# lhoyer/improving_segmentation_with_selfsupervised_depth

Measured on AMD Instinct MI355X. Metric: train images/sec, ResNet-101 joint seg+depth @512x1024, higher is better.
Workload: dtype f32

## Files before the change

### improving_segmentation_with_selfsupervised_depth_amd/_lib.py

```python
import ctypes
import os
from ctypes import c_int, c_long, c_float, c_void_p, c_size_t, c_uint64, c_int64, POINTER

_HERE = os.path.dirname(os.path.abspath(__file__))
LIB_PATH = os.environ.get("SEGSDE_LIB") or os.path.join(_HERE, "libsegsde_hip.so")
ABI_VERSION = 21

_LIB = None
HOST_POINTERS_OK = False


class PackJob(ctypes.Structure):
    _fields_ = [("w", c_void_p), ("fwd", c_void_p), ("dgrad", c_void_p)] + [(n, c_int) for n in (
        "O", "I", "KH", "KW", "block0", "reserved")]


class WinoJob(ctypes.Structure):
    _fields_ = [("w", c_void_p), ("u_fwd", c_void_p), ("u_dgrad", c_void_p)] + [(n, c_int) for n in ("O", "I", "block0", "reserved")]


class BnFoldJob(ctypes.Structure):
    _fields_ = [(n, c_void_p) for n in ("w", "cb", "gamma", "beta", "mean", "var", "w_out", "b_out")] + [("eps", c_float)] + [
        (n, c_int) for n in ("O", "I", "KH", "KW", "block0", "reserved")]

# ... 5 lines not shown


P = c_void_p
_SIGS = {
    "segsde_abi_version": (c_int, []),
    "segsde_conv_compute_taken": (c_int, [POINTER(ConvDesc), c_int]),
    "segsde_split_bf16_planes": (c_int, [P, c_long, P, P, P, P]),
    "segsde_conv2d_forward": (c_int, [POINTER(ConvDesc), P, P, P, P, P, P, P]),
    "segsde_conv2d_stats_rows": (c_long, [POINTER(ConvDesc)]),
    "segsde_conv2d_forward_stats": (c_int, [POINTER(ConvDesc), P, P, P, P, P, P, P, P]),
    "segsde_conv2d_dgrad_actgrad": (c_int, [POINTER(ConvDesc), P, P, P, P, P, P, P, P, c_int, c_int, P]),
    "segsde_bn_stats_from_partials_workspace": (c_size_t, [c_int]),
    "segsde_bn_stats_from_partials": (c_int, [P, c_long, c_long, c_int, P, P, P, P, c_float, c_float, P, P, c_size_t, P]),
    "segsde_conv2d_forward_residual": (c_int, [POINTER(ConvDesc), P, P, P, P, P, c_int, P, P]),
    "segsde_conv2d_wgrad_workspace": (c_size_t, [POINTER(ConvDesc)]),
    "segsde_conv2d_wgrad": (c_int, [POINTER(ConvDesc), P, P, P, c_int, P, P, c_size_t, P]),
    "segsde_conv2d_winograd_workspace": (c_size_t, [POINTER(ConvDesc)]),
    "segsde_conv2d_winograd_stats_rows": (ctypes.c_long, [POINTER(ConvDesc)]),
    "segsde_winograd_pack": (c_int, [P, c_int, c_int, P, P, P]),
    "segsde_winograd_pack_multi": (c_int, [P, c_int, c_int, P]),
    "segsde_conv2d_winograd": (c_int, [POINTER(ConvDesc), P, P, P, P, P, P, P, P, c_size_t, P]),
    "segsde_conv2d_wgrad_winograd_workspace": (c_size_t, [POINTER(ConvDesc)]),
    "segsde_conv2d_wgrad_winograd": (c_int, [POINTER(ConvDesc), P, P, P, c_int, P, P, P, c_size_t, P]),
    "segsde_winograd_fused_ok": (c_int, [c_int, c_int, c_int, c_int, c_int]),
    "segsde_winograd_fused_stats_rows": (ctypes.c_long, [c_int, c_int, c_int]),
    "segsde_winograd_fused_pack": (c_int, [P, c_int, c_int, c_int, P, P]),
    "segsde_conv2d_winograd_fused": (c_int, [P, c_int, c_int, c_int, c_int, c_int, c_int, P, c_int, P, c_int, P, c_int, c_int, P, P]),
    "segsde_conv2d_winograd_fused2": (c_int, [P, c_int, c_int, c_int, P, c_int, c_int, c_int, c_int, c_int, c_int, P, c_int, P, c_int, P,
                                              c_int, P, P]),
    "segsde_conv2d_winograd_fused_dgrad": (c_int, [P, c_int, c_int, c_int, c_int, c_int, P, c_int, c_int, P, c_int, c_int, P, c_int, c_int, P]),
    "segsde_reflect_adjoint_borders": (c_int, [P, P, P, P, P, c_int, c_int, P]),
    "segsde_reflect_adjoint_borders_ok": (c_int, [P, c_int]),
    "segsde_reflect_adjoint_borders2": (c_int, [P, c_int, P, c_int, P, c_int, P, c_int, c_int, c_int, c_int, c_int, c_int, c_int, P]),
    "segsde_conv2d_wgrad_winograd_fused_workspace": (c_size_t, [P]),
    "segsde_conv2d_wgrad_winograd_fused": (c_int, [P, P, P, P, c_int, P, P, c_size_t, P]),
    "segsde_upfold_pack": (c_int, [P, c_int, c_int, c_int, P, P, P]),
    "segsde_conv2d_forward_upfold": (c_int, [POINTER(ConvDesc), P, P, P, P, P, P, P]),
    "segsde_conv2d_dgrad_upfold": (c_int, [POINTER(ConvDesc), P, c_int, P, P, P, P, P, c_int, P, c_int, c_int, P]),
    "segsde_conv2d_wgrad_upfold_workspace": (c_size_t, [POINTER(ConvDesc)]),
    "segsde_conv2d_wgrad_upfold": (c_int, [POINTER(ConvDesc), P, P, P, c_int, P, P, c_size_t, P]),
    "segsde_stem_pack": (c_int, [P, c_int, c_int, c_int, P, P]),
    "segsde_stem7x7_stats_rows": (c_long, [c_int, c_int, c_int, c_int, c_int]),
    "segsde_stem7x7_forward": (c_int, [P, c_int, c_int, c_int, c_int, P, c_int, P, P, P]),
    "segsde_stem7x7_forward_bias_act": (c_int, [P, c_int, c_int, c_int, c_int, P, c_int, P, c_int, P, P]),
    "segsde_stem7x7_wgrad_workspace": (c_size_t, [c_int, c_int, c_int, c_int, c_int]),
    "segsde_stem7x7_wgrad": (c_int, [P, c_int, c_int, c_int, c_int, P, c_int, c_int, c_int, P, P, c_size_t, P]),
    "segsde_nchw_to_nhwc_bordered": (c_int, [P, c_int, c_int, c_int, c_int, c_float, c_float, P, c_int, c_int, c_int, c_int, c_int, P]),
    "segsde_pack_weight": (c_int, [P, P, c_int, c_int, c_int, c_int, c_int, P]),
    "segsde_pack_weight_both": (c_int, [P, P, P, c_int, c_int, c_int, c_int, P]),
    "segsde_pack_weight_both_multi": (c_int, [P, c_int, c_int, P]),
    "segsde_reflect_dgrad_fix": (c_int, [P, c_int, P, P, c_int, P, c_int, c_int, c_int, c_int, c_int, c_int, c_int, P]),
    "segsde_bn_stats_workspace": (c_size_t, [c_long, c_int]),
    "segsde_bn_stats": (c_int, [P, c_int, c_long, c_int, P, P, P, P, c_float, c_float, P, P, c_size_t, P]),
    "segsde_bn_eval_stats": (c_int, [P, P, c_int, c_float, P, P, P]),
    "segsde_bn_fold": (c_int, [P, c_int, c_int, P]),
    "segsde_bn_apply": (c_int, [P, c_int, c_long, c_int, P, P, P, P, P, c_int, P, c_int, c_int, c_float, c_uint64, P]),
    "segsde_bn_backward_workspace": (c_size_t, [c_long, c_int]),
    "segsde_bn_backward": (c_int, [P, c_int, P, c_int, P, c_int, c_long, c_int, P, P, P, P, c_int, c_float, c_uint64, c_int,
                                   P, P, P, c_int, P, c_int, P, c_size_t, P]),
    "segsde_bn_mask_words": (c_size_t, [c_long, c_int]),
    "segsde_bn_apply_mask": (c_int, [P, c_int, c_long, c_int, P, P, P, P, P, c_int, P, c_int, c_int, c_float, c_uint64, P, P]),
    "segsde_bn_backward_mask": (c_int, [P, c_int, P, P, c_int, c_long, c_int, P, P, P, c_int, c_float, c_int, P, P, P, c_int, P, c_int,
                                        P, c_size_t, P]),
    "segsde_colsum_workspace": (c_size_t, [c_long, c_int]),
    "segsde_act_backward": (c_int, [P, c_int, P, c_int, c_long, c_int, c_int, P, c_int, P, P, c_size_t, P]),
    "segsde_colsum": (c_int, [P, c_int, c_long, c_int, P, P, c_size_t, P]),
# ... 120 lines not shown
```

### improving_segmentation_with_selfsupervised_depth_amd/csrc/winograd_fused.hip

```cpp
#include <stdlib.h>
#include <type_traits>
#include "segsde_common.h"
#include "winograd.h"
#ifndef WINO_UP_SKIP
#define WINO_UP_SKIP 1
#endif

namespace {
#define ST(s) static_cast<hipStream_t>(s)
constexpr int FT_H = 4, FT_W = 8;
constexpr int FP_H = 2 * FT_H + 2, FP_W = 2 * FT_W + 2;
constexpr int FROW = 20, FODD = FP_W / 2;
constexpr int FPS = 256;
__device__ __forceinline__ constexpr int fplane(int c) { return c * FPS + 2 * (c >> 2); }
constexpr int FCH = 64;
constexpr int FZP = 36;
constexpr int F_FLOATS = 8 * 64 * FZP > FCH * FPS ? 8 * 64 * FZP : FCH * FPS;
#ifdef WINO_DBG_OCC1
constexpr size_t F_LDS = 96 * 1024;
#else
constexpr size_t F_LDS = (size_t)F_FLOATS * sizeof(float) + 2 * 4 * 64 * sizeof(double);
#endif

struct WinoSrc { const float* x0; const float* x1; int ld0, ld1, C0, up0; };
// ... 359 lines not shown
    }
  }
}

struct BorderP {
  const float* dy; const float* wp ; float* dx; const float* agy;
  int lddy, lddx, agld, agkind, B, H, W, Cin, Cout, mode, nseg, ldw;
};

__global__ __launch_bounds__(256) void reflect_borders_kernel(BorderP p) {
  SEGSDE_SMEM;
  float* sh = reinterpret_cast<float*>(segsde_smem);
  const int tid = threadIdx.x, lane = tid & 63, wave = tid >> 6, m = lane & 31, kk = lane >> 5;
  const int L = p.mode == 0 ? p.W : p.H;
  int r = blockIdx.x;
  const int seg = r % p.nseg; r /= p.nseg;
  const int far = r & 1, b = r >> 1;
  const int p0 = seg * 32, pitch = p.Cout + 1, cq4 = p.Cout >> 2;
  const int fixed = p.mode == 0 ? (far ? p.H - 1 : 0) : (far ? p.W - 1 : 0);
  for (int idx = tid; idx < 34 * cq4; idx += 256) {
    const int px = idx / cq4, q = idx - px * cq4, pos = p0 - 1 + px;
    float4 v = make_float4(0.f, 0.f, 0.f, 0.f);
    if (pos >= 0 && pos < L) {
      const long pix = p.mode == 0 ? ((long)(b * p.H + fixed) * p.W + pos) : ((long)(b * p.H + pos) * p.W + fixed);
      v = *reinterpret_cast<const float4*>(p.dy + pix * p.lddy + 4 * q);
    }
    float* d = sh + px * pitch + 4 * q;
    d[0] = v.x; d[1] = v.y; d[2] = v.z; d[3] = v.w;
  }
  __syncthreads();
  const int ktap = far ? 2 : 0;
  const bool top = p.mode == 1 && p0 <= 1 && 1 < p0 + 32, bot = p.mode == 1 && p0 <= p.H - 2 && p.H - 2 < p0 + 32;
  const int steps = p.Cout >> 1;
  for (int nb = wave; nb < (p.Cin >> 5); nb += 4) {
    const int cin = nb * 32 + m;
    f32x16 acc;
#pragma unroll
    for (int q = 0; q < 16; ++q) acc[q] = 0.f;
    for (int t = 0; t < 5; ++t) {
      if (t == 3 && !top) continue;
      if (t == 4 && !bot) continue;
      int kh, kw, src; bool mine = true;
      if (t < 3) {
        kh = p.mode == 0 ? ktap : t; kw = p.mode == 0 ? t : ktap; src = m + 2 - t;
      } else {
        kh = t == 3 ? 0 : 2; kw = ktap;
        const int at = t == 3 ? 1 : p.H - 2;
        mine = p0 + m == at;
        src = (t == 3 ? 0 : p.H - 1) - (p0 - 1);
      }
      const float* ap = sh + src * pitch + kk;
      const float* bp = p.wp + ((long)kk * 9 + kh * 3 + kw) * p.ldw + cin;
      const long bstep = 18L * p.ldw;
      float bv[2][8];
#pragma unroll
      for (int u = 0; u < 8; ++u) bv[0][u] = u < steps ? bp[u * bstep] : 0.f;
      for (int s0 = 0; s0 < steps; s0 += 16) {
#pragma unroll
        for (int half = 0; half < 2; ++half) {
          const int sb = s0 + 8 * half;
          if (sb < steps) {
#pragma unroll
            for (int u = 0; u < 8; ++u) bv[half ^ 1][u] = sb + 8 + u < steps ? bp[(long)(sb + 8 + u) * bstep] : 0.f;
#pragma unroll
            for (int u = 0; u < 8; ++u) {
              if (sb + u < steps) {
                const float a = mine ? ap[2 * (sb + u)] : 0.f;
// ... 78 lines not shown
                                            int Cout, const float* bias, int act, float* y, int ldy, int accumulate, double* stats,
                                            void* stream) {
  if (!x || !u_kn || !y) return SEGSDE_ERR_NULL;
  if (!segsde_winograd_fused_ok(B, H, W, C, Cout) || ldx < C || ldx % 4 != 0 || !pitch_ok(H, W, ldx) || ldy < Cout || !pitch_ok(H, W, ldy) || (accumulate && (stats || bias || act)))
    return SEGSDE_ERR_UNSUPPORTED;
  const WinoSrc src{x, nullptr, ldx, 0, C, 0};
  return launch_fused(src, B, H, W, C, reflect, u_kn, Cout, Cout, bias, act, y, ldy, accumulate, stats, WinoAg{nullptr, 0, 0}, stream);
}

extern "C" int segsde_conv2d_winograd_fused2(const float* x0, int ld0, int C0, int up0, const float* x1, int ld1, int C1, int B, int H,
                                             int W, int reflect, const float* u_kn, int Cout, const float* bias, int act, float* y,
                                             int ldy, double* stats, void* stream) {
  if (!x0 || !u_kn || !y || (C1 > 0 && !x1)) return SEGSDE_ERR_NULL;
  const int C = C0 + (C1 > 0 ? C1 : 0);
  if (!segsde_winograd_fused_ok(B, H, W, C, Cout) || C0 <= 0 || C0 % FCH || ld0 < C0 || ld0 % 4 != 0 || (C1 > 0 && (ld1 < C1 || ld1 % 4 != 0 || !pitch_ok(H, W, ld1))) ||
      !pitch_ok(H >> (up0 ? 1 : 0), W >> (up0 ? 1 : 0), ld0) || ldy < Cout || !pitch_ok(H, W, ldy))
    return SEGSDE_ERR_UNSUPPORTED;
  const WinoSrc src{x0, x1, ld0, ld1, C0, up0 ? 1 : 0};
  return launch_fused(src, B, H, W, C, reflect, u_kn, Cout, Cout, bias, act, y, ldy, 0, stats, WinoAg{nullptr, 0, 0}, stream);
}

extern "C" int segsde_conv2d_winograd_fused_dgrad(const float* dy, int lddy, int B, int H, int W, int Cout, const float* ud_kn, int ldu,
                                                  int Cin, float* dx, int lddx, int accumulate, const float* act_out, int act_ld,
                                                  int act_kind, void* stream) {
  if (!dy || !ud_kn || !dx) return SEGSDE_ERR_NULL;
  if (!segsde_winograd_fused_ok(B, H, W, Cout, Cin) || ldu < Cin || (long)16 * Cout * ldu >= (1L << 28) || lddy < Cout || lddy % 4 != 0 || !pitch_ok(H, W, lddy) || lddx < Cin || !pitch_ok(H, W, lddx) ||
      (act_out && (act_kind < SEGSDE_ACT_RELU || act_kind > SEGSDE_ACT_SIGMOID || act_ld < Cin || !pitch_ok(H, W, act_ld))))
    return SEGSDE_ERR_UNSUPPORTED;
  const WinoSrc src{dy, nullptr, lddy, 0, Cout, 0};
  return launch_fused(src, B, H, W, Cout, 0, ud_kn, ldu, Cin, nullptr, SEGSDE_ACT_NONE, dx, lddx, accumulate, nullptr,
                      WinoAg{act_out, act_ld, act_kind}, stream);
}

extern "C" int segsde_reflect_adjoint_borders2(const float* dy, int lddy, const float* wpack, int ldw, float* dx, int lddx,
                                               const float* act_out, int act_ld, int act_kind, int B, int H, int W, int Cin, int Cout,
                                               void* stream) {
  if (!dy || !wpack || !dx) return SEGSDE_ERR_NULL;
  if (B <= 0 || H < 4 || W < 4 || Cin <= 0 || Cin % 32 || ldw < Cin || Cout <= 0 || Cout % 32 || Cout > 1024 || lddy < Cout || lddy % 4 || lddx < Cin ||
      ((uintptr_t)dy & 15) || (act_out && (act_kind < SEGSDE_ACT_RELU || act_kind > SEGSDE_ACT_SIGMOID || act_ld < Cin)))
    return SEGSDE_ERR_UNSUPPORTED;
  BorderP p;
  p.dy = dy; p.wp = wpack; p.dx = dx; p.agy = act_out; p.lddy = lddy; p.lddx = lddx; p.agld = act_ld; p.agkind = act_kind;
  p.B = B; p.H = H; p.W = W; p.Cin = Cin; p.Cout = Cout; p.ldw = ldw;
  const size_t lb = (size_t)34 * (Cout + 1) * sizeof(float);
  (void)hipFuncSetAttribute(reinterpret_cast<const void*>(reflect_borders_kernel), hipFuncAttributeMaxDynamicSharedMemorySize, (int)lb);
  for (int mode = 0; mode < 2; ++mode) {
    p.mode = mode; p.nseg = ((mode == 0 ? W : H) + 31) / 32;
    hipLaunchKernelGGL(reflect_borders_kernel, dim3((unsigned)(B * 2 * p.nseg)), dim3(256), lb, ST(stream), p);
    SEGSDE_CHECK_LAUNCH();
  }
  return 0;
}
```

### improving_segmentation_with_selfsupervised_depth_amd/functional.py

```python
import collections
import weakref

import torch
from torch.autograd import Function as _TorchFunction

from . import hipops as H


class Function(_TorchFunction):

    @classmethod
    def apply(cls, *args):
        return super(_TorchFunction, cls).apply(*args)


FUSIONS = {}
BN_BITMASK = True


def _grad_dest(param):
    from . import ddp
    return ddp.grad_destination(param) if ddp._GRAD_DEST else None


# ... 144 lines not shown

    @staticmethod
    def forward(ctx, x0, x1, weight, bias, g, act, stats_out=None, grad_box=None, packs=None, x0_act=None, act_box=None,
                fold_cache=None, wino_cache=None, skip_box=None):
        ctx.grad_box = grad_box
        ctx.skip_box = skip_box
        ctx.x0_act, ctx.act_box = x0_act, act_box
        x0 = _c(x0) if x0.stride(-1) != 1 else x0
        ctx.wd = None
        ctx.wd_gen = None
        if packs is not None:
            wp, ctx.wd = packs
            ctx.wd_gen = getattr(ctx.wd, "_segsde_gen", None)
        elif ctx.needs_input_grad[0] or (x1 is not None and ctx.needs_input_grad[1]):
            wp, ctx.wd = H.pack_weight_both(weight)
        else:
            wp = H.pack_weight(weight, False)
        ctx.wp = wp if g.reflect else None
        ctx.fold = None
        ctx.wino = None
        up_f = 2 if g.up0 else 1
        kn = H.winograd_fused_ok(g, x0.shape[0], x0.shape[1] * up_f, x0.shape[2] * up_f)
        kn_d2 = (x1 is not None and g.up0 and (ctx.needs_input_grad[1])
                 and H.winograd_fused_dgrad2_ok(g, x0.shape[0], x0.shape[1] * up_f, x0.shape[2] * up_f))
        if kn or kn_d2 or (not g.up0 and H.winograd_ok(g, x0.shape[0], x0.shape[1], x0.shape[2])):
            knl = kn or kn_d2
            if (wino_cache is not None and wino_cache.get("key") is not None and wino_cache.get("key") == wino_cache.get("want")
                    and bool(wino_cache.get("kn")) == knl):
                ctx.wino = wino_cache["packs"]
            else:
                ctx.wino = H.winograd_pack(weight, kn=knl)
                if wino_cache is not None and wino_cache.get("want") is not None:
                    wino_cache["packs"], wino_cache["key"], wino_cache["kn"] = ctx.wino, wino_cache["want"], knl
        wino_f = None if (ctx.wino is None or (kn_d2 and not kn)) else ctx.wino[0]
        keep_v = wino_f is not None and not kn and ctx.needs_input_grad[2]
        H.WINO_V[0] = None
        if stats_out is not None:
            y, part = H.conv_forward(g, x0, x1, wp, bias, act, want_stats=True, wino=wino_f, keep_v=keep_v)
            stats_out.append(part)
        else:
            if H.upfold_ok(g, 4 * x0.shape[0] * x0.shape[1] * x0.shape[2]) and x0.is_contiguous() and (x1 is None or x1.is_contiguous()):
                if fold_cache is not None and fold_cache.get("key") is not None and fold_cache.get("key") == fold_cache.get("want"):
                    ctx.fold = fold_cache["fold"]
                else:
                    ctx.fold = H.upfold_pack(weight, g.C0)
                    if fold_cache is not None and fold_cache.get("want") is not None:
                        fold_cache["fold"], fold_cache["key"] = ctx.fold, fold_cache["want"]
            y = H.conv_forward(g, x0, x1, wp, bias, act, wfold=None if ctx.fold is None else ctx.fold[0], wino=wino_f, keep_v=keep_v)
        ctx.wino_v, H.WINO_V[0] = H.WINO_V[0], None
        ctx.g, ctx.act = g, act
        ctx.in_hw = (x0.shape[1] * (2 if g.up0 else 1), x0.shape[2] * (2 if g.up0 else 1))
        ctx.has_bias = bias is not None
        ctx.save_for_backward(x0, x1, weight)
        return y

    @staticmethod
    def backward(ctx, dy):
        x0, x1, weight = ctx.saved_tensors
        g = ctx.g
        dz = _c(dy)
        need_b = ctx.has_bias and ctx.needs_input_grad[3]
        dbias = None
        if need_b:
            stash = ctx.act_box.pop("dbias", None) if ctx.act_box is not None else None
            same = stash is not None and stash[0].data_ptr() == dz.data_ptr() and stash[0]._version == stash[1] == dz._version
            dbias = stash[2] if same else H.colsum(dz)
            fusion("bias_grad_from_activation_pass", bool(same))
        actgrad = (x0, ctx.x0_act) if ctx.x0_act is not None else None
        dx0 = dx1 = dw = None
        if ctx.needs_input_grad[0] or (x1 is not None and ctx.needs_input_grad[1]):
            wd = ctx.wd if ctx.wd is not None else H.pack_weight(weight, True)
            if ctx.wd_gen is not None and getattr(wd, "_segsde_gen", None) != ctx.wd_gen:
                raise RuntimeError("the weight packs of this graph were rebuilt by a later weight_pack_scope(model): a graph "
                                   "must be consumed before the next prepack of the same weights")
            dx0 = None
            box = ctx.grad_box
            if box is not None and box.get("g") is not None and x1 is None:
                dx0, dx1 = H.conv_dgrad(g, dz, wd, weight.detach(), ctx.in_hw, accumulate_into=box["g"], actgrad=actgrad,
                                        wino=None if ctx.wino is None else ctx.wino[1], wfpack=ctx.wp)
                if dx0 is not None:
                    box["fused"] = True
            if dx0 is None:
                sbox = ctx.skip_box if (x1 is not None and ctx.needs_input_grad[1]) else None
                dx0, dx1 = H.conv_dgrad(g, dz, wd, weight.detach(), ctx.in_hw, actgrad=actgrad, fold=ctx.fold,
                                        need0=ctx.needs_input_grad[0], need1=x1 is not None and ctx.needs_input_grad[1],
                                        wino=None if ctx.wino is None else ctx.wino[1],
                                        accumulate_skip_into=None if sbox is None else sbox.get("g"), wfpack=ctx.wp)
                if sbox is not None and dx1 is not None:
                    if H.SKIP_ACCUMULATED[0]:
                        sbox["fused"] = True
                    elif sbox.get("publish") and sbox.get("g") is None and dx1.is_contiguous():
                        sbox["g"] = dx1
                        sbox["fused"] = True
                if box is not None and box.get("publish") and box.get("g") is None and x1 is None and not g.up0 \
                        and dx0.is_contiguous():
                    box["g"] = dx0
                    box["fused"] = True
            if actgrad is not None and ctx.needs_input_grad[0]:
                fusion("activation_backward_in_dgrad_epilogue", bool(H.ACTGRAD_FUSED[0]))
            if not ctx.needs_input_grad[0]:
                dx0 = None
            if x1 is None or not ctx.needs_input_grad[1]:
                dx1 = None
        if ctx.needs_input_grad[2]:
            dw = H.conv_wgrad(g, x0, x1, dz, wino_v=ctx.wino_v, out=_grad_dest(weight))
            ctx.wino_v = None
        return dx0, dx1, dw, dbias, None, None, None, None, None, None, None, None, None, None


class ActGradFn(Function):

    passes = 0

    @staticmethod
    def forward(ctx, y, act, box):
        ctx.act, ctx.box = act, box
        ctx.save_for_backward(y)
        return y.view_as(y)

    @staticmethod
# ... 503 lines not shown
```

### improving_segmentation_with_selfsupervised_depth_amd/hipops.py

```python
import ctypes
import os
import threading

import numpy as np
import torch

from . import _lib
from ._lib import ConvDesc, check

ACT = {"none": 0, "relu": 1, "elu": 2, "sigmoid": 3}


class _Slot(threading.local):

    def __init__(self, default=None):
        self.default = default
        self.v = default

    def __getattr__(self, name):
        if name == "v":
            return self.__dict__.setdefault("v", self.__dict__.get("default"))
        raise AttributeError(name)

    def __getitem__(self, i):
# ... 136 lines not shown
    C1 = 0 if x1 is None else x1.shape[3]
    L = _lib.lib()
    d = ConvDesc(B=B, H=H, W=W, C0=C0, C1=C1, ld0=nhwc_ld(x0), ld1=nhwc_ld(x1) if x1 is not None else 0, up0=0, Ho=H, Wo=W,
                 Cout=Cout, ldy=Cout, ldy2=0, nsplit=0, KH=3, KW=3, stride=1, dil=g.dil, pad=g.dil,
                 pad_mode=PAD_REFLECT if reflect else PAD_ZERO, in_div=1, act=ACT[act], sum2x2=0)
    nbytes = L.segsde_conv2d_winograd_workspace(ctypes.byref(d))
    if not nbytes:
        return None
    y = torch.empty((B, H, W, Cout), dtype=torch.float32, device=x0.device)
    part = None
    if want_stats:
        part = torch.empty((int(L.segsde_conv2d_winograd_stats_rows(ctypes.byref(d))), 2, Cout), dtype=torch.float64, device=x0.device)
    ws = _ws(nbytes, x0)
    Tp = (B * (H // 2) * (W // 2) + 127) // 128 * 128
    vk = torch.empty((16, Tp, C0 + C1), dtype=torch.float32, device=x0.device) if keep_v else None
    rc = _timed(kind, flops, x0, lambda: L.segsde_conv2d_winograd(ctypes.byref(d), _p(_f32(x0)), _p(x1), _p(upack), _p(bias), _p(y),
                                                                   _p(part), _p(vk), _p(ws), nbytes, _stream(x0)), tag + " wino",
                executed=flops * 16.0 / 36.0)
    if rc == -4:
        return None
    check(rc, "conv2d_winograd")
    WINO_V[0] = vk
    WINOGRAD_TAKEN["fwd" if kind == "conv_fwd" else "dgrad"] += 1
    return y, part


WINO_FUSED = os.environ.get("SEGSDE_WINO_FUSED", "1") != "0"
WINO_FUSED_MAX_CH = int(os.environ.get("SEGSDE_WINO_FUSED_MAX_CH", "256"))
WINO_FUSED2 = os.environ.get("SEGSDE_WINO_FUSED2", "1") != "0"
WINO_UP_SKIP = os.environ.get("SEGSDE_WINO_UP_SKIP", "1") != "0"
WINO_FUSED2_MAX_CIN = int(os.environ.get("SEGSDE_WINO_FUSED2_MAX_CIN", "768"))
WINO_FUSED2_MIN_FOLD = float(os.environ.get("SEGSDE_WINO_FUSED2_MIN_FOLD", "0.6"))
WINO_FUSED_DGRAD_EXT = os.environ.get("SEGSDE_WINO_FUSED_DGRAD_EXT", "1") != "0"
WINO_FUSED_REFLECT_DGRAD_MIN_PIX = int(os.environ.get("SEGSDE_WINO_FUSED_REFLECT_DGRAD_MIN_PIX", str(1 << 17)))
WINO_FUSED_DGRAD2 = os.environ.get("SEGSDE_WINO_FUSED_DGRAD2", "1") != "0"
BORDERS2 = os.environ.get("SEGSDE_BORDERS2", "1") != "0"
WINO_FUSED_UBLK = os.environ.get("SEGSDE_WINO_FUSED_UBLK", "1") != "0"
WINO_FUSED_TAKEN = {"fwd": 0, "dgrad": 0, "fwd2": 0, "dgrad_refl": 0, "dgrad_actgrad": 0, "dgrad2": 0, "wgrad": 0}


_FUSED_SHAPE_OK = {}


def _fused_shape_ok(B, H, W, cin, cout):
    key = (B, H, W, cin, cout)
    r = _FUSED_SHAPE_OK.get(key)
    if r is None:
        r = _FUSED_SHAPE_OK[key] = bool(_lib.lib().segsde_winograd_fused_ok(B, H, W, cin, cout))
    return r


def winograd_fused_ok(g, B=None, H=None, W=None, dgrad=False):
    if g.compute == 1:
        return False
    cin, cout = (g.Cout, g.C0) if dgrad else (g.Cin, g.Cout)
    if not (WINOGRAD and WINO_FUSED and g.k == 3 and g.stride == 1 and g.dil == 1 and g.pad == 1 and g.cin_alg is None
            and cin % 64 == 0 and cout % 64 == 0):
        return False
    if g.up0 or g.C1:
        if dgrad or not (WINO_FUSED2 and g.up0 and g.C0 % 64 == 0 and cin <= WINO_FUSED2_MAX_CIN and cout <= WINO_FUSED_MAX_CH
                         and _fold_frac(g) >= WINO_FUSED2_MIN_FOLD):
            return False
    else:
        if max(cin, cout) > WINO_FUSED_MAX_CH or (dgrad and g.reflect and not WINO_FUSED_DGRAD_EXT):
            return False
    if B is None:
        return True
    return _fused_shape_ok(B, H, W, cin, cout) and 9.0 * B * H * W * cin * cout >= WINOGRAD_MIN_MACS


def winograd_fused_dgrad2_ok(g, B=None, H=None, W=None):
    if g.compute == 1:
        return False
    if not (WINOGRAD and WINO_FUSED and WINO_FUSED_DGRAD_EXT and WINO_FUSED_DGRAD2 and BORDERS2 and g.k == 3 and g.stride == 1 and g.dil == 1
            and g.pad == 1 and g.reflect and g.up0 and g.C1 and g.cin_alg is None and g.C1 % 64 == 0 and g.Cout % 64 == 0
            and g.C0 % 64 == 0
            and g.Cout <= WINO_FUSED_MAX_CH and g.Cin <= WINO_FUSED2_MAX_CIN):
        return False
    if B is None:
        return True
    return (B * H * W >= WINO_FUSED_REFLECT_DGRAD_MIN_PIX and _fused_shape_ok(B, H, W, g.Cout, g.C1)
            and 9.0 * B * H * W * g.C1 * g.Cout >= WINOGRAD_MIN_MACS)


def winograd_fused_static_ok(conv):
    if not (WINOGRAD and WINO_FUSED and conv.kernel_size == (3, 3) and conv.stride == (1, 1) and conv.padding == (1, 1)
            and conv.dilation == (1, 1) and conv.in_channels % 64 == 0 and conv.out_channels % 64 == 0):
        return False
    if max(conv.in_channels, conv.out_channels) <= WINO_FUSED_MAX_CH:
        return True
    return bool(WINO_FUSED2 and getattr(conv, "reflect", False) and conv.out_channels <= WINO_FUSED_MAX_CH
                and conv.in_channels <= WINO_FUSED2_MAX_CIN)


class _KnPack(torch.Tensor):
    """a transformed weight pack of the one-kernel route: 16 K N floats, logical shape [16][K][N], stored in the blocked order the
    kernel reads (WINO_FUSED_UBLK; the sixteen [K][N] planes with SEGSDE_WINO_FUSED_UBLK=0) -- a plain tensor with a type the
    dispatch can see; only the library's pack and convolution kernels interpret its contents"""


def _kn(t):
    return t.as_subclass(_KnPack)


def winograd_fused_pack(w_oihw, flip):
    O, I = w_oihw.shape[0], w_oihw.shape[1]
    w = _f32(w_oihw.detach()).contiguous()
    u = torch.empty((16, O, I) if flip else (16, I, O), dtype=torch.float32, device=w.device)
    check(_lib.lib().segsde_winograd_fused_pack(_p(w), O, I, 1 if flip else 0, _p(u), _stream(w)), "winograd_fused_pack")
    return _kn(u)


def winograd_fused(kind, x, u_kn, bias=None, act="none", want_stats=False, tag=None, reflect=False, accumulate_into=None, x1=None,
                   up0=False, actgrad=None, adjoint=None, cols=None):
    B, H0, W0, C0 = x.shape
    H, W = (2 * H0, 2 * W0) if up0 else (H0, W0)
    C1 = 0 if x1 is None else x1.shape[3]
    C = C0 + C1
    ldu = u_kn.shape[2]
    n_off, N = (0, ldu) if cols is None else cols
    assert u_kn.shape[1] == C and n_off + N <= ldu and (cols is None or (actgrad is not None or adjoint is not None or kind == "conv_dgrad"))
    L = _lib.lib()
    if accumulate_into is not None:
        y = accumulate_into
        if tuple(y.shape) != (B, H, W, N) or not y.is_contiguous() or bias is not None or act != "none" or want_stats:
            return None
    else:
        y = torch.empty((B, H, W, N), dtype=torch.float32, device=x.device)
    part = None
    if want_stats:
        part = torch.empty((int(L.segsde_winograd_fused_stats_rows(B, H, W)), 2, N), dtype=torch.float64, device=x.device)
    flops = 2.0 * B * H * W * C * N * 9
    tagf = (tag or "%d+%d->%d k3 s1 d1 %dx%d" % (C0, C1, N, H, W)) + " wino-fused"
    if x1 is not None or up0:
        assert accumulate_into is None and actgrad is None and adjoint is None
        rc = _timed(kind, flops, x, lambda: L.segsde_conv2d_winograd_fused2(
            _p(_f32(x)), nhwc_ld(x), C0, 1 if up0 else 0, _p(x1), nhwc_ld(x1) if x1 is not None else 0, C1, B, H, W, 1 if reflect else 0,
            _p(u_kn), N, _p(bias), ACT[act], _p(y), N, _p(part), _stream(x)), tagf,
            executed=flops * ((9.0 * C0 + 16.0 * C1) / (36.0 * (C0 + C1)) if (up0 and WINO_UP_SKIP) else 16.0 / 36.0))
        if rc == -4:
            return None
        check(rc, "conv2d_winograd_fused2")
        WINO_FUSED_TAKEN["fwd2"] += 1
        return y, part
    if actgrad is not None or adjoint is not None or cols is not None:
        assert bias is None and act == "none" and not want_stats and not reflect
        ag_y, ag_kind = (actgrad[0], ACT[actgrad[1]]) if actgrad is not None else (None, 0)
        ag_ld = nhwc_ld(ag_y) if ag_y is not None else 0
        acc = 1 if accumulate_into is not None else 0
        d = wdpack = wfpack = None
        if adjoint is not None:
            g, wdpack, wfpack = adjoint
            if wfpack is None or not BORDERS2:
                assert cols is None
                d = _borders_desc(B, H, W, C, N, nhwc_ld(x))

        def launch():
            u_off = 4 * ((n_off // 64) * 256 if WINO_FUSED_UBLK else n_off)
            rc = L.segsde_conv2d_winograd_fused_dgrad(_p(_f32(x)), nhwc_ld(x), B, H, W, C, ctypes.c_void_p(u_kn.data_ptr() + u_off), ldu,
                                                      N, _p(y), N, acc, _p(ag_y), ag_ld, ag_kind, _stream(x))
            if rc == 0 and adjoint is not None:
                if d is None:
                    rc = L.segsde_reflect_adjoint_borders2(_p(x), nhwc_ld(x), ctypes.c_void_p(wfpack.data_ptr() + 4 * n_off), wfpack.shape[3],
                                                           _p(y), N, _p(ag_y), ag_ld, ag_kind, B, H, W, N, C, _stream(x))
                else:
                    rc = L.segsde_reflect_adjoint_borders(ctypes.byref(d), _p(x), _p(wdpack), _p(y), _p(ag_y), ag_ld, ag_kind, _stream(x))
                if rc == -4:
                    raise RuntimeError("the mirrored-padding launches declined a shape the one-kernel data-gradient took: "
                                       "the zero-padded part is already in dx (hipops.conv_dgrad must gate this)")
            return rc
        rc = _timed(kind, flops, x, launch, tagf, executed=flops * 16.0 / 36.0)
        if rc == -4:
            return None
        check(rc, "conv2d_winograd_fused_dgrad")
        WINO_FUSED_TAKEN["dgrad"] += 1
        WINO_FUSED_TAKEN["dgrad_refl"] += adjoint is not None
        WINO_FUSED_TAKEN["dgrad_actgrad"] += actgrad is not None
        return y, None
    rc = _timed(kind, flops, x, lambda: L.segsde_conv2d_winograd_fused(_p(_f32(x)), nhwc_ld(x), B, H, W, C, 1 if reflect else 0, _p(u_kn), N, _p(bias),
                                                                       ACT[act], _p(y), N, 1 if accumulate_into is not None else 0, _p(part), _stream(x)),
                tagf, executed=flops * 16.0 / 36.0)
    if rc == -4:
        return None
    check(rc, "conv2d_winograd_fused")
    WINO_FUSED_TAKEN["fwd" if kind == "conv_fwd" else "dgrad"] += 1
    return y, part


def _borders_desc(B, H, W, Cout, Cin, lddy):
    return ConvDesc(B=B, H=H, W=W, C0=Cout, C1=0, ld0=lddy, ld1=0, up0=0, Ho=H, Wo=W, Cout=Cin, ldy=Cin, ldy2=0, nsplit=Cin, KH=3, KW=3,
                    stride=1, dil=1, pad=1, pad_mode=PAD_REFLECT_ADJOINT, in_div=1, act=0, sum2x2=0, accumulate=1)


def reflect_borders_ok(B, H, W, Cout, Cin, lddy, ag_ld=0):
    return bool(_lib.lib().segsde_reflect_adjoint_borders_ok(ctypes.byref(_borders_desc(B, H, W, Cout, Cin, lddy)), int(ag_ld)))


WINO_FUSED_WGRAD = os.environ.get("SEGSDE_WINO_FUSED_WGRAD", "1") != "0"
WINO_FUSED_WGRAD_MAX_CH = int(os.environ.get("SEGSDE_WINO_FUSED_WGRAD_MAX_CH", "256"))
WINO_FUSED_WGRAD_MAX_CIN2 = int(os.environ.get("SEGSDE_WINO_FUSED_WGRAD_MAX_CIN2", "768"))
WINO_FUSED_WGRAD_MIN_FOLD = float(os.environ.get("SEGSDE_WINO_FUSED_WGRAD_MIN_FOLD", "0.4"))


def winograd_fused_wgrad_ok(g, B=None, H=None, W=None):
    if g.compute == 1:
        return False
    if not (WINOGRAD and WINO_FUSED and WINO_FUSED_WGRAD and g.k == 3 and g.stride == 1 and g.dil == 1 and g.pad == 1
            and g.cin_alg is None and g.C0 % 32 == 0 and g.C1 % 32 == 0 and g.Cout % 64 == 0 and g.Cout <= WINO_FUSED_WGRAD_MAX_CH):
        return False
# ... 205 lines not shown
        r = _winograd("conv_fwd", g, x0, x1, wino, g.Cout, want_stats, flops, _tag(g, H, W), bias=bias, act=act, reflect=g.reflect,
                      keep_v=keep_v and WINOGRAD_KEEP_V)
        if r is not None:
            return r if want_stats else r[0]
    if wfold is not None and not want_stats:
        rc = _timed("conv_fwd", flops, x0, lambda: _lib.lib().segsde_conv2d_forward_upfold(
            ctypes.byref(d), _p(_f32(x0)), _p(x1), _p(wpack), _p(wfold), _p(bias), _p(y), _stream(x0)), _tag(g, H, W) + " fold",
            executed=flops * _fold_frac(g))
        if rc == 0:
            UPFOLD_TAKEN["fwd"] += 1
            _note_compute(d, 4, "fwd")
            return y
        if rc != -4:
            check(rc, "conv2d_forward_upfold")
    part = None
    if want_stats and bias is None and act == "none":
        rows = int(_lib.lib().segsde_conv2d_stats_rows(ctypes.byref(d)))
        if rows > 0:
            part = torch.empty((rows, 2, g.Cout), dtype=torch.float64, device=x0.device)
    _timed("conv_fwd", flops, x0, lambda: check(_lib.lib().segsde_conv2d_forward_stats(
        ctypes.byref(d), _p(_f32(x0)), _p(x1), _p(wpack), _p(bias), _p(y), None, _p(part), _stream(x0)), "conv2d_forward"),
        _tag(g, H, W), executed=flops_x)
    _note_compute(d, 0, "fwd")
    return (y, part) if want_stats else y


ACTGRAD_FUSED = _Slot(False)


SKIP_ACCUMULATED = _Slot(False)


def conv_dgrad(g, dy, wdpack, w_oihw, in_hw, need0=True, need1=True, accumulate_into=None, actgrad=None, fold=None, wino=None,
               accumulate_skip_into=None, wfpack=None):
    B, Ho, Wo, Cout = dy.shape
    H, W = in_hw
    assert Cout == g.Cout
    ACTGRAD_FUSED[0] = False
    SKIP_ACCUMULATED[0] = False
    dx1 = torch.empty((B, H, W, g.C1), dtype=torch.float32, device=dy.device) if g.C1 else None
    L = _lib.lib()
    flops = 2.0 * B * Ho * Wo * Cout * g.CinAlg * g.k * g.k
    ag_y, ag_ld, ag_kind = None, 0, 0
    if actgrad is not None:
        ag_y, ag_kind = actgrad[0], ACT[actgrad[1]]
        ag_ld = nhwc_ld(ag_y)

    if isinstance(wino, _KnPack):
        ext = actgrad is not None or g.reflect
        if (winograd_fused_ok(g, B, H, W, dgrad=True) and (Ho, Wo) == (H, W) and (not ext or WINO_FUSED_DGRAD_EXT)
                and (not g.reflect or B * H * W >= WINO_FUSED_REFLECT_DGRAD_MIN_PIX)
                and (not g.reflect or (wfpack is not None and BORDERS2 and H >= 4 and W >= 4 and g.C0 % 32 == 0 and Cout % 32 == 0 and Cout <= 1024)
                     or reflect_borders_ok(B, H, W, Cout, g.C0, nhwc_ld(dy), ag_ld))
                and (actgrad is None or (ag_ld % 4 == 0 and ag_y.data_ptr() % 16 == 0))):
            r = winograd_fused("conv_dgrad", dy, wino, tag=_tag(g, H, W), accumulate_into=accumulate_into, actgrad=actgrad,
                               adjoint=(g, wdpack, wfpack) if g.reflect else None)
            if r is not None:
                ACTGRAD_FUSED[0] = actgrad is not None
                return r[0], None
    elif (wino is not None and accumulate_into is None and actgrad is None and not g.reflect and g.C1 == 0
            and winograd_ok(g, B, H, W, dgrad=True) and (Ho, Wo) == (H, W)):
        r = _winograd("conv_dgrad", g, dy, None, wino, g.C0, False, flops, _tag(g, H, W))
        if r is not None:
            return r[0], None

    def desc(sum2x2, accumulate=0):
        return ConvDesc(B=B, H=Ho, W=Wo, C0=Cout, C1=0, ld0=nhwc_ld(dy), ld1=0, up0=0, Ho=H, Wo=W, Cout=g.Cin, ldy=g.C0,
                        ldy2=g.C1, nsplit=g.C0, KH=g.k, KW=g.k, stride=1, dil=g.dil, pad=(g.k - 1) * g.dil - g.pad,
                        pad_mode=PAD_REFLECT_ADJOINT if g.reflect else PAD_ZERO, in_div=g.stride, act=0, sum2x2=sum2x2,
                        accumulate=accumulate, compute=g.compute)

    def launch(d, y, y2, fuse):
        return L.segsde_conv2d_dgrad_actgrad(ctypes.byref(d), _p(_f32(dy)), None, _p(wdpack), None, _p(y), _p(y2), None,
                                             _p(ag_y) if fuse else None, ag_ld if fuse else 0, ag_kind if fuse else 0,
                                             _stream(dy))

    def finish_unfused(dx0):
        if actgrad is None or dx0 is None:
            return dx0
        dz, _ = act_backward(dx0, ag_y, actgrad[1])
        return dz

    if accumulate_into is not None:
        acc = accumulate_into
        if g.up0 or g.C1 or tuple(acc.shape) != (B, H, W, g.C0) or not acc.is_contiguous():
            return None, None
        d = desc(0, 1)
        rc = _timed("conv_dgrad", flops, dy, lambda: launch(d, acc, None, actgrad is not None), _tag(g, H, W),
                    executed=flops * _live_tap_frac(g, H, W))
        if rc == -4:
            return None, None
        check(rc, "conv2d dgrad (accumulate)")
        _note_compute(d, 1, "dgrad")
        ACTGRAD_FUSED[0] = actgrad is not None
        return acc, None
    if g.up0 and fold is not None and accumulate_into is None:
        wfold, wdfold = fold
# ... 1249 lines not shown
```

### include/segsde_hip.h

```cpp
#ifndef SEGSDE_HIP_H
#define SEGSDE_HIP_H
#include <stddef.h>
#include <stdint.h>

#ifdef __cplusplus
extern "C" {
#endif

#define SEGSDE_ABI_VERSION 21

enum { SEGSDE_ERR_NULL = -1, SEGSDE_ERR_SHAPE = -2, SEGSDE_ERR_WORKSPACE = -3, SEGSDE_ERR_UNSUPPORTED = -4 };
enum { SEGSDE_ACT_NONE = 0, SEGSDE_ACT_RELU = 1, SEGSDE_ACT_ELU = 2, SEGSDE_ACT_SIGMOID = 3 };
enum { SEGSDE_DTYPE_F32 = 0, SEGSDE_DTYPE_I64 = 1, SEGSDE_DTYPE_U8 = 2 };
enum { SEGSDE_PAD_ZERO = 0, SEGSDE_PAD_REFLECT = 1, SEGSDE_PAD_REFLECT_ADJOINT = 2 };

int segsde_abi_version(void);

typedef struct segsde_conv_desc {
  int B, H, W;
  int C0, C1;
  int ld0, ld1;
  int up0;
  int Ho, Wo, Cout;
  int ldy, ldy2, nsplit;
// ... 126 lines not shown
int segsde_nchw_to_nhwc_bordered(const float* x, int B, int C, int H, int W, float mean, float sd, float* y, int ldy, int pad_top,
                                 int pad_left, int Hp, int Wp, void* stream);
int segsde_nhwc_to_nchw(const float* x, int ldx, int B, int C, int H, int W, float* y, void* stream);

typedef struct segsde_wino_job {
  const float* w;
  float* u_fwd;
  float* u_dgrad;
  int O, I, block0, reserved;
} segsde_wino_job;
size_t segsde_conv2d_winograd_workspace(const segsde_conv_desc* d);
long segsde_conv2d_winograd_stats_rows(const segsde_conv_desc* d);
int segsde_winograd_pack(const float* w_oihw, int Cout, int Cin, float* u_fwd, float* u_dgrad, void* stream);
int segsde_winograd_pack_multi(const segsde_wino_job* jobs_device, int njobs, int total_blocks, void* stream);
int segsde_conv2d_winograd(const segsde_conv_desc* d, const float* x0, const float* x1, const float* u_pack, const float* bias,
                           float* y, double* stats, float* v_keep, void* workspace, size_t workspace_bytes, void* stream);
size_t segsde_conv2d_wgrad_winograd_workspace(const segsde_conv_desc* d);
int segsde_conv2d_wgrad_winograd(const segsde_conv_desc* d, const float* x0, const float* x1, const float* dy, int lddy,
                                 const float* v_saved, float* dw_oihw, void* workspace, size_t workspace_bytes, void* stream);
int segsde_winograd_fused_ok(int B, int H, int W, int C, int Cout);
long segsde_winograd_fused_stats_rows(int B, int H, int W);
int segsde_winograd_fused_pack(const float* w_oihw, int Cout, int Cin, int flip, float* u_kn, void* stream);
int segsde_conv2d_winograd_fused(const float* x, int ldx, int B, int H, int W, int C, int reflect, const float* u_kn, int Cout,
                                 const float* bias, int act, float* y, int ldy, int accumulate, double* stats, void* stream);
int segsde_conv2d_winograd_fused2(const float* x0, int ld0, int C0, int up0, const float* x1, int ld1, int C1, int B, int H, int W,
                                  int reflect, const float* u_kn, int Cout, const float* bias, int act, float* y, int ldy,
                                  double* stats, void* stream);
int segsde_conv2d_winograd_fused_dgrad(const float* dy, int lddy, int B, int H, int W, int Cout, const float* ud_kn, int ldu, int Cin,
                                       float* dx, int lddx, int accumulate, const float* act_out, int act_ld, int act_kind, void* stream);
int segsde_reflect_adjoint_borders(const segsde_conv_desc* d, const float* dy, const float* wdpack, float* y, const float* act_out,
                                   int act_ld, int act_kind, void* stream);
int segsde_reflect_adjoint_borders2(const float* dy, int lddy, const float* wpack, int ldw, float* dx, int lddx, const float* act_out,
                                    int act_ld, int act_kind, int B, int H, int W, int Cin, int Cout, void* stream);
int segsde_reflect_adjoint_borders_ok(const segsde_conv_desc* d, int act_ld);
size_t segsde_conv2d_wgrad_winograd_fused_workspace(const segsde_conv_desc* d);
int segsde_conv2d_wgrad_winograd_fused(const segsde_conv_desc* d, const float* x0, const float* x1, const float* dy, int lddy,
                                       float* dw_oihw, void* workspace, size_t workspace_bytes, void* stream);

int segsde_pose_matrix_forward(const float* axisangle, const float* translation, int B, int stride, int invert, float* M,
                               void* stream);
int segsde_pose_matrix_backward(const float* axisangle, const float* translation, const float* dM, int B, int stride,
                                int invert, float* daxisangle, float* dtranslation, void* stream);

int segsde_warp_forward(const float* disp, int hs, int ws, const float* inv_K, const float* K, const float* T,
                        const float* src, int B, int H, int W, float min_depth, float max_depth, float* color,
                        float* grid, float* depth, void* stream);
size_t segsde_warp_backward_workspace(int B, int H, int W);
int segsde_warp_backward(const float* gcolor, const float* disp, int hs, int ws, const float* inv_K, const float* K,
                         const float* T, const float* src, int B, int H, int W, float min_depth, float max_depth,
                         float* g_disp_up, float* gT, void* workspace, size_t workspace_bytes, void* stream);
int segsde_reprojection_error_forward(const float* pred, const float* target, int B, int H, int W, int no_ssim,
                                      float* err, long err_bstride, void* stream);
size_t segsde_reprojection_error_backward_workspace(int B, int H, int W);
int segsde_reprojection_error_backward(const float* pred, const float* target, const float* gerr, long gerr_bstride, int B,
                                       int H, int W, int no_ssim, float* gpred, void* workspace, size_t workspace_bytes,
                                       void* stream);
size_t segsde_automask_workspace(int B, int H, int W);
int segsde_automask_min_forward(const float* ident, const float* noise, const float* reproj, int n_reproj, int avg, int B,
                                int H, int W, uint8_t* sel, float* identity_selection, float* sum_out, void* workspace,
                                size_t workspace_bytes, void* stream);
int segsde_automask_min_backward(const uint8_t* sel, int n_ident, int n_reproj, int avg, int B, int H, int W, float scale,
                                 float* greproj, void* stream);
size_t segsde_smoothness_workspace(int B, int h, int w);
int segsde_smoothness_forward(const float* disp, const float* img, int B, int h, int w, float* mean_disp, float* out,
                              void* workspace, size_t workspace_bytes, void* stream);
int segsde_smoothness_backward(const float* disp, const float* img, const float* mean_disp, int B, int h, int w,
// ... 114 lines not shown
```

Measured before the change: 64.24.

## Add flat fused Winograd dgrad path for concat-input reflect convs and split border kernel

Adds a dgrad path for reflect-padded 3x3 convs with two concatenated inputs (decoder skip concat). It packs a flat fused Winograd weight, cached alongside the existing packs, and runs the fused dgrad kernel twice over column ranges, one for the main input and one for the skip input, accumulating into the skip gradient directly. The reflect-border adjoint kernel now spreads its input-channel blocks across a second grid dimension to raise parallelism. The minimum pixel threshold for fused reflect dgrad is lowered so smaller layers also take the fused path. The cost is an extra weight pack and cache entry per layer, and two kernel launches where there was one generic dgrad.

```diff
diff --git a/improving_segmentation_with_selfsupervised_depth_amd/_lib.py b/improving_segmentation_with_selfsupervised_depth_amd/_lib.py
--- a/improving_segmentation_with_selfsupervised_depth_amd/_lib.py
+++ b/improving_segmentation_with_selfsupervised_depth_amd/_lib.py
@@ -61,6 +61,8 @@
     "segsde_reflect_adjoint_borders": (c_int, [P, P, P, P, P, c_int, c_int, P]),
     "segsde_reflect_adjoint_borders_ok": (c_int, [P, c_int]),
     "segsde_reflect_adjoint_borders2": (c_int, [P, c_int, P, c_int, P, c_int, P, c_int, c_int, c_int, c_int, c_int, c_int, c_int, P]),
+    "segsde_reflect_adjoint_borders2_split": (c_int, [P, c_int, P, c_int, P, c_int, P, c_int, c_int, c_int, c_int, c_int, c_int, c_int, c_int,
+                                                      P]),
     "segsde_conv2d_wgrad_winograd_fused_workspace": (c_size_t, [P]),
     "segsde_conv2d_wgrad_winograd_fused": (c_int, [P, P, P, P, c_int, P, P, c_size_t, P]),
     "segsde_upfold_pack": (c_int, [P, c_int, c_int, c_int, P, P, P]),
diff --git a/improving_segmentation_with_selfsupervised_depth_amd/csrc/winograd_fused.hip b/improving_segmentation_with_selfsupervised_depth_amd/csrc/winograd_fused.hip
--- a/improving_segmentation_with_selfsupervised_depth_amd/csrc/winograd_fused.hip
+++ b/improving_segmentation_with_selfsupervised_depth_amd/csrc/winograd_fused.hip
@@ -415,7 +415,7 @@
   const int ktap = far ? 2 : 0;
   const bool top = p.mode == 1 && p0 <= 1 && 1 < p0 + 32, bot = p.mode == 1 && p0 <= p.H - 2 && p.H - 2 < p0 + 32;
   const int steps = p.Cout >> 1;
-  for (int nb = wave; nb < (p.Cin >> 5); nb += 4) {
+  for (int nb = 4 * blockIdx.y + wave; nb < (p.Cin >> 5); nb += 4 * gridDim.y) {
     const int cin = nb * 32 + m;
     f32x16 acc;
 #pragma unroll
@@ -560,9 +560,9 @@
                       WinoAg{act_out, act_ld, act_kind}, stream);
 }
 
-extern "C" int segsde_reflect_adjoint_borders2(const float* dy, int lddy, const float* wpack, int ldw, float* dx, int lddx,
-                                               const float* act_out, int act_ld, int act_kind, int B, int H, int W, int Cin, int Cout,
-                                               void* stream) {
+extern "C" int segsde_reflect_adjoint_borders2_split(const float* dy, int lddy, const float* wpack, int ldw, float* dx, int lddx,
+                                                     const float* act_out, int act_ld, int act_kind, int B, int H, int W, int Cin,
+                                                     int Cout, int split, void* stream) {
   if (!dy || !wpack || !dx) return SEGSDE_ERR_NULL;
   if (B <= 0 || H < 4 || W < 4 || Cin <= 0 || Cin % 32 || ldw < Cin || Cout <= 0 || Cout % 32 || Cout > 1024 || lddy < Cout || lddy % 4 || lddx < Cin ||
       ((uintptr_t)dy & 15) || (act_out && (act_kind < SEGSDE_ACT_RELU || act_kind > SEGSDE_ACT_SIGMOID || act_ld < Cin)))
@@ -572,10 +572,17 @@
   p.B = B; p.H = H; p.W = W; p.Cin = Cin; p.Cout = Cout; p.ldw = ldw;
   const size_t lb = (size_t)34 * (Cout + 1) * sizeof(float);
   (void)hipFuncSetAttribute(reinterpret_cast<const void*>(reflect_borders_kernel), hipFuncAttributeMaxDynamicSharedMemorySize, (int)lb);
+  const unsigned groups = split ? (unsigned)((Cin / 32 + 3) / 4) : 1u;
   for (int mode = 0; mode < 2; ++mode) {
     p.mode = mode; p.nseg = ((mode == 0 ? W : H) + 31) / 32;
-    hipLaunchKernelGGL(reflect_borders_kernel, dim3((unsigned)(B * 2 * p.nseg)), dim3(256), lb, ST(stream), p);
+    hipLaunchKernelGGL(reflect_borders_kernel, dim3((unsigned)(B * 2 * p.nseg), groups), dim3(256), lb, ST(stream), p);
     SEGSDE_CHECK_LAUNCH();
   }
   return 0;
 }
+
+extern "C" int segsde_reflect_adjoint_borders2(const float* dy, int lddy, const float* wpack, int ldw, float* dx, int lddx,
+                                               const float* act_out, int act_ld, int act_kind, int B, int H, int W, int Cin, int Cout,
+                                               void* stream) {
+  return segsde_reflect_adjoint_borders2_split(dy, lddy, wpack, ldw, dx, lddx, act_out, act_ld, act_kind, B, H, W, Cin, Cout, 1, stream);
+}
diff --git a/improving_segmentation_with_selfsupervised_depth_amd/functional.py b/improving_segmentation_with_selfsupervised_depth_amd/functional.py
--- a/improving_segmentation_with_selfsupervised_depth_amd/functional.py
+++ b/improving_segmentation_with_selfsupervised_depth_amd/functional.py
@@ -200,6 +200,17 @@
                 ctx.wino = H.winograd_pack(weight, kn=knl)
                 if wino_cache is not None and wino_cache.get("want") is not None:
                     wino_cache["packs"], wino_cache["key"], wino_cache["kn"] = ctx.wino, wino_cache["want"], knl
+        ctx.wino_flat = None
+        if (x1 is not None and not g.up0 and (ctx.needs_input_grad[0] or ctx.needs_input_grad[1])
+                and H.winograd_fused_dgrad2_flat_ok(g, x0.shape[0], x0.shape[1], x0.shape[2])):
+            want = wino_cache.get("want") if wino_cache is not None else None
+            hit = wino_cache.get("flat") if want is not None else None
+            if hit is not None and hit[0] == want:
+                ctx.wino_flat = hit[1]
+            else:
+                ctx.wino_flat = H.winograd_fused_pack(weight, True)
+                if want is not None:
+                    wino_cache["flat"] = (want, ctx.wino_flat)
         wino_f = None if (ctx.wino is None or (kn_d2 and not kn)) else ctx.wino[0]
         keep_v = wino_f is not None and not kn and ctx.needs_input_grad[2]
         H.WINO_V[0] = None
@@ -253,7 +264,8 @@
                 dx0, dx1 = H.conv_dgrad(g, dz, wd, weight.detach(), ctx.in_hw, actgrad=actgrad, fold=ctx.fold,
                                         need0=ctx.needs_input_grad[0], need1=x1 is not None and ctx.needs_input_grad[1],
                                         wino=None if ctx.wino is None else ctx.wino[1],
-                                        accumulate_skip_into=None if sbox is None else sbox.get("g"), wfpack=ctx.wp)
+                                        accumulate_skip_into=None if sbox is None else sbox.get("g"), wfpack=ctx.wp,
+                                        wino_flat=ctx.wino_flat)
                 if sbox is not None and dx1 is not None:
                     if H.SKIP_ACCUMULATED[0]:
                         sbox["fused"] = True
diff --git a/improving_segmentation_with_selfsupervised_depth_amd/hipops.py b/improving_segmentation_with_selfsupervised_depth_amd/hipops.py
--- a/improving_segmentation_with_selfsupervised_depth_amd/hipops.py
+++ b/improving_segmentation_with_selfsupervised_depth_amd/hipops.py
@@ -192,11 +192,12 @@
 WINO_FUSED2_MAX_CIN = int(os.environ.get("SEGSDE_WINO_FUSED2_MAX_CIN", "768"))
 WINO_FUSED2_MIN_FOLD = float(os.environ.get("SEGSDE_WINO_FUSED2_MIN_FOLD", "0.6"))
 WINO_FUSED_DGRAD_EXT = os.environ.get("SEGSDE_WINO_FUSED_DGRAD_EXT", "1") != "0"
-WINO_FUSED_REFLECT_DGRAD_MIN_PIX = int(os.environ.get("SEGSDE_WINO_FUSED_REFLECT_DGRAD_MIN_PIX", str(1 << 17)))
+WINO_FUSED_REFLECT_DGRAD_MIN_PIX = int(os.environ.get("SEGSDE_WINO_FUSED_REFLECT_DGRAD_MIN_PIX", str(1 << 13)))
 WINO_FUSED_DGRAD2 = os.environ.get("SEGSDE_WINO_FUSED_DGRAD2", "1") != "0"
+WINO_FUSED_DGRAD2_FLAT = os.environ.get("SEGSDE_WINO_FUSED_DGRAD2_FLAT", "1") != "0"
 BORDERS2 = os.environ.get("SEGSDE_BORDERS2", "1") != "0"
 WINO_FUSED_UBLK = os.environ.get("SEGSDE_WINO_FUSED_UBLK", "1") != "0"
-WINO_FUSED_TAKEN = {"fwd": 0, "dgrad": 0, "fwd2": 0, "dgrad_refl": 0, "dgrad_actgrad": 0, "dgrad2": 0, "wgrad": 0}
+WINO_FUSED_TAKEN = {"fwd": 0, "dgrad": 0, "fwd2": 0, "dgrad_refl": 0, "dgrad_actgrad": 0, "dgrad2": 0, "dgrad2_flat": 0, "wgrad": 0}
 
 
 _FUSED_SHAPE_OK = {}
@@ -243,6 +244,19 @@
             and 9.0 * B * H * W * g.C1 * g.Cout >= WINOGRAD_MIN_MACS)
 
 
+def winograd_fused_dgrad2_flat_ok(g, B=None, H=None, W=None):
+    if g.compute == 1:
+        return False
+    if not (WINOGRAD and WINO_FUSED and WINO_FUSED_DGRAD_EXT and WINO_FUSED_DGRAD2_FLAT and BORDERS2 and g.k == 3 and g.stride == 1
+            and g.dil == 1 and g.pad == 1 and g.reflect and g.C1 and not g.up0 and g.cin_alg is None and g.C0 % 64 == 0
+            and g.C1 % 64 == 0 and g.Cout % 64 == 0 and g.Cout <= WINO_FUSED_MAX_CH and 16 * g.Cout * g.Cin < (1 << 28)):
+        return False
+    if B is None:
+        return True
+    return (B * H * W >= WINO_FUSED_REFLECT_DGRAD_MIN_PIX and _fused_shape_ok(B, H, W, g.Cout, g.C0) and _fused_shape_ok(B, H, W, g.Cout, g.C1)
+            and 9.0 * B * H * W * g.Cin * g.Cout >= WINOGRAD_MIN_MACS)
+
+
 def winograd_fused_static_ok(conv):
     if not (WINOGRAD and WINO_FUSED and conv.kernel_size == (3, 3) and conv.stride == (1, 1) and conv.padding == (1, 1)
             and conv.dilation == (1, 1) and conv.in_channels % 64 == 0 and conv.out_channels % 64 == 0):
@@ -272,7 +286,7 @@
 
 
 def winograd_fused(kind, x, u_kn, bias=None, act="none", want_stats=False, tag=None, reflect=False, accumulate_into=None, x1=None,
-                   up0=False, actgrad=None, adjoint=None, cols=None):
+                   up0=False, actgrad=None, adjoint=None, cols=None, counted=True):
     B, H0, W0, C0 = x.shape
     H, W = (2 * H0, 2 * W0) if up0 else (H0, W0)
     C1 = 0 if x1 is None else x1.shape[3]
@@ -333,8 +347,8 @@
         if rc == -4:
             return None
         check(rc, "conv2d_winograd_fused_dgrad")
-        WINO_FUSED_TAKEN["dgrad"] += 1
-        WINO_FUSED_TAKEN["dgrad_refl"] += adjoint is not None
+        WINO_FUSED_TAKEN["dgrad"] += bool(counted)
+        WINO_FUSED_TAKEN["dgrad_refl"] += adjoint is not None and bool(counted)
         WINO_FUSED_TAKEN["dgrad_actgrad"] += actgrad is not None
         return y, None
     rc = _timed(kind, flops, x, lambda: L.segsde_conv2d_winograd_fused(_p(_f32(x)), nhwc_ld(x), B, H, W, C, 1 if reflect else 0, _p(u_kn), N, _p(bias),
@@ -606,7 +620,7 @@
 
 
 def conv_dgrad(g, dy, wdpack, w_oihw, in_hw, need0=True, need1=True, accumulate_into=None, actgrad=None, fold=None, wino=None,
-               accumulate_skip_into=None, wfpack=None):
+               accumulate_skip_into=None, wfpack=None, wino_flat=None):
     B, Ho, Wo, Cout = dy.shape
     H, W = in_hw
     assert Cout == g.Cout
@@ -637,6 +651,26 @@
         r = _winograd("conv_dgrad", g, dy, None, wino, g.C0, False, flops, _tag(g, H, W))
         if r is not None:
             return r[0], None
+
+    if (isinstance(wino_flat, _KnPack) and wfpack is not None and accumulate_into is None and (Ho, Wo) == (H, W)
+            and winograd_fused_dgrad2_flat_ok(g, B, H, W) and (actgrad is None or (ag_ld % 4 == 0 and ag_y.data_ptr() % 16 == 0))
+            and (need0 or need1)):
+        acc1 = accumulate_skip_into
+        if not (need1 and acc1 is not None and tuple(acc1.shape) == (B, H, W, g.C1) and acc1.is_contiguous()):
+            acc1 = None
+        r0 = r1 = None
+        tagp = "k3 s1 d1 %dx%d refl %s-of-%d+%d"
+        if need0:
+            r0 = winograd_fused("conv_dgrad", dy, wino_flat, tag="%d+0->%d " % (Cout, g.C0) + tagp % (H, W, "first", g.C0, g.C1),
+                                actgrad=actgrad, adjoint=(g, wdpack, wfpack), cols=(0, g.C0))
+        if (r0 is not None or not need0) and need1:
+            r1 = winograd_fused("conv_dgrad", dy, wino_flat, tag="%d+0->%d " % (Cout, g.C1) + tagp % (H, W, "skip", g.C0, g.C1),
+                                accumulate_into=acc1, adjoint=(g, wdpack, wfpack), cols=(g.C0, g.C1), counted=r0 is None)
+        if (r0 is not None or not need0) and (r1 is not None or not need1):
+            WINO_FUSED_TAKEN["dgrad2_flat"] += 1
+            ACTGRAD_FUSED[0] = actgrad is not None and r0 is not None
+            SKIP_ACCUMULATED[0] = acc1 is not None
+            return (None if r0 is None else r0[0]), (None if r1 is None else r1[0])
 
     def desc(sum2x2, accumulate=0):
         return ConvDesc(B=B, H=Ho, W=Wo, C0=Cout, C1=0, ld0=nhwc_ld(dy), ld1=0, up0=0, Ho=H, Wo=W, Cout=g.Cin, ldy=g.C0,
diff --git a/include/segsde_hip.h b/include/segsde_hip.h
--- a/include/segsde_hip.h
+++ b/include/segsde_hip.h
@@ -182,6 +182,9 @@
                                    int act_ld, int act_kind, void* stream);
 int segsde_reflect_adjoint_borders2(const float* dy, int lddy, const float* wpack, int ldw, float* dx, int lddx, const float* act_out,
                                     int act_ld, int act_kind, int B, int H, int W, int Cin, int Cout, void* stream);
+int segsde_reflect_adjoint_borders2_split(const float* dy, int lddy, const float* wpack, int ldw, float* dx, int lddx,
+                                          const float* act_out, int act_ld, int act_kind, int B, int H, int W, int Cin, int Cout,
+                                          int split, void* stream);
 int segsde_reflect_adjoint_borders_ok(const segsde_conv_desc* d, int act_ld);
 size_t segsde_conv2d_wgrad_winograd_fused_workspace(const segsde_conv_desc* d);
 int segsde_conv2d_wgrad_winograd_fused(const segsde_conv_desc* d, const float* x0, const float* x1, const float* dy, int lddy,
```

Result: no change. 64.84, median of 6 (+0.9%).
